# chinhau5/parallel_eda

Hardware: AMD Instinct MI355X
Metric: place+route wall-clock to feasibility (s/flow; bitcoin_miner-scale synthetic on stratixiv-like fabric) (lower is better)
Workload: dtype fp32; 1 GPU; model=bitcoin_miner, arch=bitcoin_stratixiv, grid=280x200, W=300, rr_nodes=15745036, rr_edges=87277236, blocks=37632, nets=35616, conns=110426, global_batch=110426, seq_len=0, final_overused=0, wirelength=4914365

## Files before the change

csrc/hip/place_kernel.hip:

```cpp
#include "pnr_hip.h"

namespace pnrh {

struct PlaceDev {
  const int32_t* net_blk_ptr;
  const int32_t* net_blks;
  const int32_t* blk_net_ptr;
  const int32_t* blk_nets;
  const int8_t* blk_type;
  const int8_t* tile_btype;
  const int32_t* type_cols;
  const int32_t* type_col_ptr;
  const uint8_t* fixed;
  const float* net_q;
  const int32_t* net_sink_ptr;
  const float* conn_crit;
  const float* delay_mat;
  int32_t* bx;
  int32_t* by;
  int32_t* bslot;
  int32_t* grid;
  float* net_cost;
  float* net_tcost;
  int32_t num_blocks, num_nets, gx, gy, cap, nx, ny, io_cap;
// ... 390 lines not shown
  }
}

__launch_bounds__(64 * PROP_WAVES, 2)
__global__ void place_apply_kernel(PlaceDev p, MovesDev m, float timing_tradeoff,
                                   double* cost_acc ) {
  const int lane = threadIdx.x & 63;
  const int i = blockIdx.x * PROP_WAVES + (threadIdx.x >> 6);
  if (i >= m.n_moves || m.mv_flags[i] != 2) return;
  int32_t blk = m.mv_blk[i];
  int32_t other = m.mv_other[i];
  int32_t to = m.mv_to[i];
  if (other <= -2) {
    const int mid = -2 - other;
    const int ddx = (to >> 13) - 4096, ddy = (to & 0x1FFF) - 4096;
    const int32_t mm0 = p.macro_ptr[mid], mm1 = p.macro_ptr[mid + 1];
    for (int32_t j = mm0; j < mm1; ++j) {
      int32_t b = p.macro_blk[j];
      for (int32_t k = p.blk_net_ptr[b] + lane; k < p.blk_net_ptr[b + 1];
           k += 64) {
        int32_t n = p.blk_nets[k];
        p.net_cost[n] = net_bb_cost_macro(p, n, mid, ddx, ddy);
        if (timing_tradeoff > 0.0f)
          p.net_tcost[n] = net_td_cost_macro(p, n, mid, ddx, ddy);
      }
    }
    if (lane == 0) {
      for (int32_t j = mm0; j < mm1; ++j) {
        int32_t b = p.macro_blk[j];
        p.grid[((int64_t)p.bx[b] * p.gy + p.by[b]) * p.cap + p.bslot[b]] = -1;
      }
      for (int32_t j = mm0; j < mm1; ++j) {
        int32_t b = p.macro_blk[j];
        int tx = p.bx[b] + ddx, ty = p.by[b] + ddy;
        p.grid[((int64_t)tx * p.gy + ty) * p.cap] = b;
        p.bx[b] = tx; p.by[b] = ty; p.bslot[b] = 0;
      }
      unsafeAtomicAdd(&cost_acc[0], (double)m.mv_dbb[i]);
      unsafeAtomicAdd(&cost_acc[1], (double)m.mv_dtd[i]);
    }
    return;
  }
  int slot1 = to % p.cap;
  int x1 = to / p.cap / p.gy, y1 = (to / p.cap) % p.gy;
  int x0 = p.bx[blk], y0 = p.by[blk], s0 = p.bslot[blk];
  const int ox = other >= 0 ? x0 : -1000, oy = other >= 0 ? y0 : -1000;
  for (int32_t k = p.blk_net_ptr[blk] + lane; k < p.blk_net_ptr[blk + 1];
       k += 64) {
    int32_t n = p.blk_nets[k];
    p.net_cost[n] = net_bb_cost(p, n, blk, x1, y1, other, ox, oy);
    if (timing_tradeoff > 0.0f)
      p.net_tcost[n] = net_td_cost(p, n, blk, x1, y1, other, ox, oy);
  }
  if (other >= 0)
    for (int32_t k = p.blk_net_ptr[other] + lane;
         k < p.blk_net_ptr[other + 1]; k += 64) {
      int32_t n = p.blk_nets[k];
      p.net_cost[n] = net_bb_cost(p, n, blk, x1, y1, other, ox, oy);
      if (timing_tradeoff > 0.0f)
        p.net_tcost[n] = net_td_cost(p, n, blk, x1, y1, other, ox, oy);
    }
  if (lane == 0) {
    p.grid[((int64_t)x0 * p.gy + y0) * p.cap + s0] = other >= 0 ? other : -1;
    p.grid[((int64_t)x1 * p.gy + y1) * p.cap + slot1] = blk;
    p.bx[blk] = x1; p.by[blk] = y1; p.bslot[blk] = slot1;
    if (other >= 0) { p.bx[other] = x0; p.by[other] = y0; p.bslot[other] = s0; }
    unsafeAtomicAdd(&cost_acc[0], (double)m.mv_dbb[i]);
    unsafeAtomicAdd(&cost_acc[1], (double)m.mv_dtd[i]);
  }
}

__global__ void place_reset_claims_kernel(int32_t* net_claim, int32_t nn,
                                          int32_t* loc_claim, int32_t nl,
                                          int32_t* counters) {
  int i = blockIdx.x * blockDim.x + threadIdx.x;
  int total = max(nn, nl);
  (void)counters;
  for (; i < total; i += gridDim.x * blockDim.x) {
    if (i < nn) net_claim[i] = 0x7FFFFFFF;
    if (i < nl) loc_claim[i] = 0x7FFFFFFF;
  }
}

struct RunDev {
  int32_t* mv_from;
  unsigned long long* net_claim;
  unsigned long long* loc_claim;
  int32_t* ctrl;
};

__device__ __forceinline__ unsigned long long claim_key(uint32_t batch, int i) {
  return ((unsigned long long)batch << 32) | (0xFFFFFFFFu - (uint32_t)i);
}

__launch_bounds__(64 * PROP_WAVES, 2)
__global__ void place_propose_run_kernel(PlaceDev p, MovesDev m, RunDev r,
                                         float T, int rlim,
                                         float timing_tradeoff,
                                         float inv_bb_norm, float inv_td_norm,
                                         uint32_t seed, uint32_t batch) {
  if (r.ctrl[0]) return;
  const int lane = threadIdx.x & 63;
  const int i = blockIdx.x * PROP_WAVES + (threadIdx.x >> 6);
  if (i >= m.n_moves) return;
  const unsigned long long key = claim_key(batch, i);
  int sel = -1, sx1 = -1, sy1 = -1, sslot = 0;
  if (lane == 0) {
    m.mv_flags[i] = 0;
    sel = propose_select_impl(p, rlim, seed, batch, i, sx1, sy1, sslot);
  }
  sel = __shfl(sel, 0);
  if (sel < 0) return;
  const int x1 = __shfl(sx1, 0);
  const int y1 = __shfl(sy1, 0);
  const int slot1 = __shfl(sslot, 0);
  const int32_t blk = sel;
  const int x0 = p.bx[blk], y0 = p.by[blk];
  const int mid = p.macro_of ? p.macro_of[blk] : -1;
  if (mid >= 0) {
    const int ddx = x1 - x0, ddy = y1 - y0;
    const int32_t mm0 = p.macro_ptr[mid], mm1 = p.macro_ptr[mid + 1];
    if (mm1 - mm0 > 16) return;
    int ok = 0;
    if (lane == 0) {
      ok = 1;
      for (int32_t j = mm0; j < mm1 && ok; ++j) {
        int32_t b = p.macro_blk[j];
        int sx = p.bx[b], sy = p.by[b];
        int tx = sx + ddx, ty = sy + ddy;
        if (p.fixed && p.fixed[b]) ok = 0;
        else if (tx < 0 || tx >= p.gx || ty < 0 || ty >= p.gy) ok = 0;
        else if (p.rx0 >= 0 && (tx < p.rx0 || tx > p.rx1 ||
                                sx < p.rx0 || sx > p.rx1)) ok = 0;
        else if (p.tile_btype
                     ? (p.tile_btype[tx * p.gy + ty] != p.blk_type[b])
                     : (is_io_loc(p, tx, ty) != (p.blk_type[b] == 0))) ok = 0;
        else if (cap_at(p, tx, ty) != 1) ok = 0;
        else {
          int32_t occ = p.grid[((int64_t)tx * p.gy + ty) * p.cap];
          if (occ >= 0 && p.macro_of[occ] != mid) ok = 0;
        }
      }
      if (ok) atomicAdd(&m.counters[0], 1);
    }
    ok = __shfl(ok, 0);
    if (!ok) return;
    float dbb = 0.0f, dtd = 0.0f;
    for (int32_t j = mm0; j < mm1; ++j) {
      int32_t b = p.macro_blk[j];
      for (int32_t k = p.blk_net_ptr[b] + lane; k < p.blk_net_ptr[b + 1];
           k += 64) {
        int32_t n = p.blk_nets[k];
        bool dup = false;
        for (int32_t j2 = mm0; j2 < j && !dup; ++j2)
          dup = blk_has_net(p, p.macro_blk[j2], n);
        if (dup) continue;
        dbb += net_bb_cost_macro(p, n, mid, ddx, ddy) - p.net_cost[n];
        if (timing_tradeoff > 0.0f)
          dtd += net_td_cost_macro(p, n, mid, ddx, ddy) - p.net_tcost[n];
      }
    }
    dbb = wave_sum_f32(dbb);
    dtd = wave_sum_f32(dtd);
    float delta = (1.0f - timing_tradeoff) * dbb * inv_bb_norm +
                  timing_tradeoff * dtd * inv_td_norm;
    bool accept;
    if (delta <= 0.0f) accept = true;
    else if (T <= 0.0f) accept = false;
    else {
      float u = (rng_hash(seed, batch, i * 131 + 5) & 0xFFFFFF) *
                (1.0f / 16777216.0f);
      accept = u < __expf(-delta / T);
    }
    if (!accept) return;
    if (lane == 0) {
      atomicAdd(&m.counters[1], 1);
      m.mv_blk[i] = blk;
      m.mv_to[i] = ((ddx + 4096) << 13) | (ddy + 4096);
      m.mv_other[i] = -2 - mid;
      m.mv_dbb[i] = dbb;
      m.mv_dtd[i] = dtd;
      m.mv_flags[i] = 1;
      r.mv_from[i] = x0 * p.gy + y0;
    }
    for (int32_t j = mm0; j < mm1; ++j) {
      int32_t b = p.macro_blk[j];
      for (int32_t k = p.blk_net_ptr[b] + lane; k < p.blk_net_ptr[b + 1];
           k += 64)
        atomicMax(&r.net_claim[p.blk_nets[k]], key);
    }
    for (int32_t j = mm0 + lane; j < mm1; j += 64) {
      int32_t b = p.macro_blk[j];
      atomicMax(&r.loc_claim[p.bx[b] * p.gy + p.by[b]], key);
      atomicMax(&r.loc_claim[(p.bx[b] + ddx) * p.gy + p.by[b] + ddy], key);
    }
    return;
  }
  int32_t other = p.grid[((int64_t)x1 * p.gy + y1) * p.cap + slot1];
  if (other == blk) return;
  if (other >= 0 && p.fixed && p.fixed[other]) return;
  if (other >= 0 && p.macro_of && p.macro_of[other] >= 0)
    return;
  if (lane == 0) atomicAdd(&m.counters[0], 1);
  float dbb = 0.0f, dtd = 0.0f;
  const int ox = other >= 0 ? x0 : -1000, oy = other >= 0 ? y0 : -1000;
  for (int32_t k = p.blk_net_ptr[blk] + lane; k < p.blk_net_ptr[blk + 1];
       k += 64) {
    int32_t n = p.blk_nets[k];
    dbb += net_bb_cost(p, n, blk, x1, y1, other, ox, oy) - p.net_cost[n];
    if (timing_tradeoff > 0.0f)
      dtd += net_td_cost(p, n, blk, x1, y1, other, ox, oy) - p.net_tcost[n];
  }
  if (other >= 0) {
    for (int32_t k = p.blk_net_ptr[other] + lane;
         k < p.blk_net_ptr[other + 1]; k += 64) {
      int32_t n = p.blk_nets[k];
      if (blk_has_net(p, blk, n)) continue;
      dbb += net_bb_cost(p, n, blk, x1, y1, other, ox, oy) - p.net_cost[n];
      if (timing_tradeoff > 0.0f)
        dtd += net_td_cost(p, n, blk, x1, y1, other, ox, oy) - p.net_tcost[n];
    }
  }
  dbb = wave_sum_f32(dbb);
  dtd = wave_sum_f32(dtd);
  float delta = (1.0f - timing_tradeoff) * dbb * inv_bb_norm +
                timing_tradeoff * dtd * inv_td_norm;
  bool accept;
  if (delta <= 0.0f) accept = true;
  else if (T <= 0.0f) accept = false;
  else {
    float u = (rng_hash(seed, batch, i * 131 + 5) & 0xFFFFFF) *
              (1.0f / 16777216.0f);
    accept = u < __expf(-delta / T);
  }
  if (!accept) return;
  if (lane == 0) {
    atomicAdd(&m.counters[1], 1);
    m.mv_blk[i] = blk;
    m.mv_to[i] = ((x1 * p.gy + y1) * p.cap + slot1);
    m.mv_other[i] = other;
    m.mv_dbb[i] = dbb;
    m.mv_dtd[i] = dtd;
    m.mv_flags[i] = 1;
    r.mv_from[i] = x0 * p.gy + y0;
    atomicMax(&r.loc_claim[x0 * p.gy + y0], key);
    atomicMax(&r.loc_claim[x1 * p.gy + y1], key);
  }
  for (int32_t k = p.blk_net_ptr[blk] + lane; k < p.blk_net_ptr[blk + 1];
       k += 64)
    atomicMax(&r.net_claim[p.blk_nets[k]], key);
  if (other >= 0)
    for (int32_t k = p.blk_net_ptr[other] + lane;
         k < p.blk_net_ptr[other + 1]; k += 64)
      atomicMax(&r.net_claim[p.blk_nets[k]], key);
}

__device__ void commit_move(const PlaceDev& p, const MovesDev& m,
                            const RunDev& r, float timing_tradeoff,
                            double* cost_acc, uint32_t batch) {
  const int lane = threadIdx.x & 63;
  const int i = blockIdx.x * PROP_WAVES + (threadIdx.x >> 6);
  if (i >= m.n_moves || m.mv_flags[i] != 1) return;
  const unsigned long long key = claim_key(batch, i);
  int32_t blk = m.mv_blk[i];
  int32_t other = m.mv_other[i];
  int32_t to = m.mv_to[i];
  bool bad = false;
  if (other <= -2) {
    const int mid = -2 - other;
    const int ddx = (to >> 13) - 4096, ddy = (to & 0x1FFF) - 4096;
    const int32_t mm0 = p.macro_ptr[mid], mm1 = p.macro_ptr[mid + 1];
    for (int32_t j = mm0 + lane; j < mm1; j += 64) {
      int32_t b = p.macro_blk[j];
      int sx = p.bx[b], sy = p.by[b];
      int tx = sx + ddx, ty = sy + ddy;
      if (tx < 0 || tx >= p.gx || ty < 0 || ty >= p.gy) bad = true;
      else if (r.loc_claim[sx * p.gy + sy] != key ||
               r.loc_claim[tx * p.gy + ty] != key) bad = true;
    }
    for (int32_t j = mm0; j < mm1; ++j) {
      int32_t b = p.macro_blk[j];
      for (int32_t k = p.blk_net_ptr[b] + lane; k < p.blk_net_ptr[b + 1];
           k += 64)
        if (r.net_claim[p.blk_nets[k]] != key) bad = true;
    }
  } else {
    int x1 = to / p.cap / p.gy, y1 = (to / p.cap) % p.gy;
    if (lane == 0 && (r.loc_claim[r.mv_from[i]] != key ||
                      r.loc_claim[x1 * p.gy + y1] != key)) bad = true;
    for (int32_t k = p.blk_net_ptr[blk] + lane; k < p.blk_net_ptr[blk + 1];
         k += 64)
      if (r.net_claim[p.blk_nets[k]] != key) bad = true;
    if (other >= 0)
      for (int32_t k = p.blk_net_ptr[other] + lane;
           k < p.blk_net_ptr[other + 1]; k += 64)
        if (r.net_claim[p.blk_nets[k]] != key) bad = true;
  }
  const bool win = !__any(bad);
  if (lane == 0) {
    if (!win) { m.mv_flags[i] = 0; atomicAdd(&m.counters[3], 1); }
    else { m.mv_flags[i] = 2; atomicAdd(&m.counters[2], 1); }
  }
  if (!win) return;
  if (other <= -2) {
    const int mid = -2 - other;
    const int ddx = (to >> 13) - 4096, ddy = (to & 0x1FFF) - 4096;
    const int32_t mm0 = p.macro_ptr[mid], mm1 = p.macro_ptr[mid + 1];
    for (int32_t j = mm0; j < mm1; ++j) {
      int32_t b = p.macro_blk[j];
      for (int32_t k = p.blk_net_ptr[b] + lane; k < p.blk_net_ptr[b + 1];
           k += 64) {
        int32_t n = p.blk_nets[k];
        p.net_cost[n] = net_bb_cost_macro(p, n, mid, ddx, ddy);
        if (timing_tradeoff > 0.0f)
          p.net_tcost[n] = net_td_cost_macro(p, n, mid, ddx, ddy);
      }
    }
    if (lane == 0) {
      for (int32_t j = mm0; j < mm1; ++j) {
        int32_t b = p.macro_blk[j];
        p.grid[((int64_t)p.bx[b] * p.gy + p.by[b]) * p.cap + p.bslot[b]] = -1;
      }
      for (int32_t j = mm0; j < mm1; ++j) {
        int32_t b = p.macro_blk[j];
        int tx = p.bx[b] + ddx, ty = p.by[b] + ddy;
        p.grid[((int64_t)tx * p.gy + ty) * p.cap] = b;
        p.bx[b] = tx; p.by[b] = ty; p.bslot[b] = 0;
      }
      unsafeAtomicAdd(&cost_acc[0], (double)m.mv_dbb[i]);
      unsafeAtomicAdd(&cost_acc[1], (double)m.mv_dtd[i]);
    }
    return;
  }
  int slot1 = to % p.cap;
  int x1 = to / p.cap / p.gy, y1 = (to / p.cap) % p.gy;
  int x0 = p.bx[blk], y0 = p.by[blk], s0 = p.bslot[blk];
  const int ox = other >= 0 ? x0 : -1000, oy = other >= 0 ? y0 : -1000;
  for (int32_t k = p.blk_net_ptr[blk] + lane; k < p.blk_net_ptr[blk + 1];
       k += 64) {
    int32_t n = p.blk_nets[k];
    p.net_cost[n] = net_bb_cost(p, n, blk, x1, y1, other, ox, oy);
    if (timing_tradeoff > 0.0f)
      p.net_tcost[n] = net_td_cost(p, n, blk, x1, y1, other, ox, oy);
  }
  if (other >= 0)
    for (int32_t k = p.blk_net_ptr[other] + lane;
         k < p.blk_net_ptr[other + 1]; k += 64) {
      int32_t n = p.blk_nets[k];
      p.net_cost[n] = net_bb_cost(p, n, blk, x1, y1, other, ox, oy);
      if (timing_tradeoff > 0.0f)
        p.net_tcost[n] = net_td_cost(p, n, blk, x1, y1, other, ox, oy);
    }
  if (lane == 0) {
    p.grid[((int64_t)x0 * p.gy + y0) * p.cap + s0] = other >= 0 ? other : -1;
    p.grid[((int64_t)x1 * p.gy + y1) * p.cap + slot1] = blk;
    p.bx[blk] = x1; p.by[blk] = y1; p.bslot[blk] = slot1;
    if (other >= 0) { p.bx[other] = x0; p.by[other] = y0; p.bslot[other] = s0; }
    unsafeAtomicAdd(&cost_acc[0], (double)m.mv_dbb[i]);
    unsafeAtomicAdd(&cost_acc[1], (double)m.mv_dtd[i]);
  }
}

__launch_bounds__(64 * PROP_WAVES, 2)
__global__ void place_commit_kernel(PlaceDev p, MovesDev m, RunDev r,
                                    float timing_tradeoff, double* cost_acc,
                                    uint32_t batch, int check,
                                    int32_t target_moves) {
  if (r.ctrl[0]) return;
  commit_move(p, m, r, timing_tradeoff, cost_acc, batch);
  if (!check) return;
  asm volatile("s_waitcnt vmcnt(0)" ::: "memory");
  __syncthreads();
  if (threadIdx.x != 0) return;
  __threadfence();
  asm volatile("s_waitcnt vmcnt(0)" ::: "memory");
  int ticket = __hip_atomic_fetch_add(&r.ctrl[2], 1, __ATOMIC_RELAXED,
                                      __HIP_MEMORY_SCOPE_AGENT);
  if (ticket != (int)gridDim.x - 1) return;
  __threadfence();
  int att = __hip_atomic_load(&m.counters[0], __ATOMIC_RELAXED,
                              __HIP_MEMORY_SCOPE_AGENT);
  int acc = __hip_atomic_load(&m.counters[1], __ATOMIC_RELAXED,
                              __HIP_MEMORY_SCOPE_AGENT);
  int win = __hip_atomic_load(&m.counters[2], __ATOMIC_RELAXED,
                              __HIP_MEMORY_SCOPE_AGENT);
  r.ctrl[1] += 4;
  if (win + (att - acc) >= target_moves) r.ctrl[0] = 1;
  __hip_atomic_store(&r.ctrl[2], 0, __ATOMIC_RELAXED,
                     __HIP_MEMORY_SCOPE_AGENT);
}

__global__ void place_refresh_costs_kernel(PlaceDev p, float timing_tradeoff,
                                           double* out ) {
  int n = blockIdx.x * blockDim.x + threadIdx.x;
  for (; n < p.num_nets; n += gridDim.x * blockDim.x) {
    float c = net_bb_cost(p, n, -1, 0, 0, -1, 0, 0);
    p.net_cost[n] = c;
    unsafeAtomicAdd(&out[0], (double)c);
    float t = (timing_tradeoff > 0.0f)
                  ? net_td_cost(p, n, -1, 0, 0, -1, 0, 0) : 0.0f;
    p.net_tcost[n] = t;
    unsafeAtomicAdd(&out[1], (double)t);
  }
}

}

using namespace pnrh;

extern "C" {

struct PlaceLaunchArgs {
  const int32_t* net_blk_ptr; const int32_t* net_blks;
  const int32_t* blk_net_ptr; const int32_t* blk_nets;
  const int8_t* blk_type; const int8_t* tile_btype;
  const int32_t* type_cols; const int32_t* type_col_ptr;
  const uint8_t* fixed;
  const float* net_q;
  const int32_t* net_sink_ptr; const float* conn_crit; const float* delay_mat;
  int32_t* bx; int32_t* by; int32_t* bslot; int32_t* grid;
  float* net_cost; float* net_tcost;
  int32_t num_blocks, num_nets, gx, gy, cap, nx, ny, io_cap;
  int32_t rx0, rx1;
  const int32_t* macro_of; const int32_t* macro_ptr;
  const int32_t* macro_blk;
  int32_t* mv_blk; int32_t* mv_to; int32_t* mv_other;
  float* mv_dbb; float* mv_dtd; uint8_t* mv_flags;
  int32_t* net_claim; int32_t* loc_claim; int32_t* counters;
  int32_t n_moves;
  float T; int32_t rlim; float timing_tradeoff;
  float inv_bb_norm, inv_td_norm;
  uint32_t seed, batch;
  double* cost_acc;
  int32_t* mv_from;
  unsigned long long* net_claim64; unsigned long long* loc_claim64;
  int32_t* run_ctrl;
};

static void unpack(const PlaceLaunchArgs* a, PlaceDev& p, MovesDev& m) {
  p.net_blk_ptr = a->net_blk_ptr; p.net_blks = a->net_blks;
  p.blk_net_ptr = a->blk_net_ptr; p.blk_nets = a->blk_nets;
  p.blk_type = a->blk_type; p.tile_btype = a->tile_btype;
  p.type_cols = a->type_cols; p.type_col_ptr = a->type_col_ptr;
  p.fixed = a->fixed;
  p.net_q = a->net_q;
  p.net_sink_ptr = a->net_sink_ptr; p.conn_crit = a->conn_crit;
  p.delay_mat = a->delay_mat;
  p.bx = a->bx; p.by = a->by; p.bslot = a->bslot; p.grid = a->grid;
  p.net_cost = a->net_cost; p.net_tcost = a->net_tcost;
  p.num_blocks = a->num_blocks; p.num_nets = a->num_nets;
  p.gx = a->gx; p.gy = a->gy; p.cap = a->cap;
  p.nx = a->nx; p.ny = a->ny; p.io_cap = a->io_cap;
  p.rx0 = a->rx0; p.rx1 = a->rx1;
  p.macro_of = a->macro_of; p.macro_ptr = a->macro_ptr;
  p.macro_blk = a->macro_blk;
  m.mv_blk = a->mv_blk; m.mv_to = a->mv_to; m.mv_other = a->mv_other;
  m.mv_dbb = a->mv_dbb; m.mv_dtd = a->mv_dtd; m.mv_flags = a->mv_flags;
  m.net_claim = a->net_claim; m.loc_claim = a->loc_claim;
  m.counters = a->counters; m.n_moves = a->n_moves;
}

int pnr_place_batch(const PlaceLaunchArgs* a, void* stream) {
  PlaceDev p; MovesDev m;
  unpack(a, p, m);
  hipStream_t s = (hipStream_t)stream;
  int rg = (max(max(a->num_nets, a->gx * a->gy), a->n_moves) + 255) / 256;
  rg = rg < 2048 ? rg : 2048;
  hipLaunchKernelGGL(place_reset_claims_kernel, dim3(rg), dim3(256), 0, s,
                     m.net_claim, p.num_nets, m.loc_claim, p.gx * p.gy,
                     m.counters);
  int mg = (m.n_moves + PROP_WAVES - 1) / PROP_WAVES;
  hipLaunchKernelGGL(place_propose_kernel, dim3(mg), dim3(64 * PROP_WAVES),
                     0, s, p, m, a->T, a->rlim, a->timing_tradeoff,
                     a->inv_bb_norm, a->inv_td_norm, a->seed, a->batch);
  hipLaunchKernelGGL(place_resolve_kernel, dim3(mg), dim3(64 * PROP_WAVES),
                     0, s, p, m);
  hipLaunchKernelGGL(place_apply_kernel, dim3(mg), dim3(64 * PROP_WAVES),
                     0, s, p, m, a->timing_tradeoff, a->cost_acc);
  return (int)hipGetLastError();
}

int pnr_place_run(const PlaceLaunchArgs* a, uint32_t first_batch,
                  int32_t target_moves, int32_t n_batches, void* stream) {
  if (n_batches < 0 || (n_batches & 3) || first_batch == 0 ||
      !a->mv_from || !a->net_claim64 || !a->loc_claim64 || !a->run_ctrl)
    return (int)hipErrorInvalidValue;
  PlaceDev p; MovesDev m;
  unpack(a, p, m);
  RunDev r;
  r.mv_from = a->mv_from;
  r.net_claim = a->net_claim64; r.loc_claim = a->loc_claim64;
  r.ctrl = a->run_ctrl;
  hipStream_t s = (hipStream_t)stream;
  int mg = (m.n_moves + PROP_WAVES - 1) / PROP_WAVES;
  for (int32_t k = 0; k < n_batches; ++k) {
    const uint32_t batch = first_batch + (uint32_t)k;
    hipLaunchKernelGGL(place_propose_run_kernel, dim3(mg),
                       dim3(64 * PROP_WAVES), 0, s, p, m, r, a->T, a->rlim,
                       a->timing_tradeoff, a->inv_bb_norm, a->inv_td_norm,
                       a->seed, batch);
    hipLaunchKernelGGL(place_commit_kernel, dim3(mg), dim3(64 * PROP_WAVES),
                       0, s, p, m, r, a->timing_tradeoff, a->cost_acc, batch,
                       (int)(((k + 1) & 3) == 0), target_moves);
  }
  return (int)hipGetLastError();
}

int pnr_place_refresh(const PlaceLaunchArgs* a, void* stream) {
  PlaceDev p; MovesDev m;
  unpack(a, p, m);
  hipStream_t s = (hipStream_t)stream;
  hipLaunchKernelGGL(place_refresh_costs_kernel, dim3(1024), dim3(256), 0, s,
                     p, a->timing_tradeoff, a->cost_acc);
  return (int)hipGetLastError();
}

int64_t pnr_place_args_sizeof() { return (int64_t)sizeof(PlaceLaunchArgs); }

}
```

parallel_eda_amd/place/gpu_placer.py:

```python
import ctypes as ct
import math

import numpy as np

from ..arch.archdef import ArchDef
from ..ops import hip_api
from .placer import Placement, analytic_delay_matrix


class PlaceLaunchArgs(ct.Structure):
    _fields_ = [
        ("net_blk_ptr", ct.c_void_p), ("net_blks", ct.c_void_p),
        ("blk_net_ptr", ct.c_void_p), ("blk_nets", ct.c_void_p),
        ("blk_type", ct.c_void_p), ("tile_btype", ct.c_void_p),
        ("type_cols", ct.c_void_p), ("type_col_ptr", ct.c_void_p),
        ("fixed", ct.c_void_p),
        ("net_q", ct.c_void_p),
        ("net_sink_ptr", ct.c_void_p), ("conn_crit", ct.c_void_p),
        ("delay_mat", ct.c_void_p),
        ("bx", ct.c_void_p), ("by", ct.c_void_p), ("bslot", ct.c_void_p),
        ("grid", ct.c_void_p),
        ("net_cost", ct.c_void_p), ("net_tcost", ct.c_void_p),
        ("num_blocks", ct.c_int32), ("num_nets", ct.c_int32),
        ("gx", ct.c_int32), ("gy", ct.c_int32), ("cap", ct.c_int32),
        ("nx", ct.c_int32), ("ny", ct.c_int32), ("io_cap", ct.c_int32),
        ("rx0", ct.c_int32), ("rx1", ct.c_int32),
        ("macro_of", ct.c_void_p), ("macro_ptr", ct.c_void_p),
        ("macro_blk", ct.c_void_p),
        ("mv_blk", ct.c_void_p), ("mv_to", ct.c_void_p), ("mv_other", ct.c_void_p),
        ("mv_dbb", ct.c_void_p), ("mv_dtd", ct.c_void_p), ("mv_flags", ct.c_void_p),
        ("net_claim", ct.c_void_p), ("loc_claim", ct.c_void_p),
        ("counters", ct.c_void_p), ("n_moves", ct.c_int32),
        ("T", ct.c_float), ("rlim", ct.c_int32), ("timing_tradeoff", ct.c_float),
        ("inv_bb_norm", ct.c_float), ("inv_td_norm", ct.c_float),
        ("seed", ct.c_uint32), ("batch", ct.c_uint32),
        ("cost_acc", ct.c_void_p),
        ("mv_from", ct.c_void_p),
        ("net_claim64", ct.c_void_p), ("loc_claim64", ct.c_void_p),
        ("run_ctrl", ct.c_void_p),
    ]


RUN_CHUNK_BATCHES = 32


def _lib():
    lib = hip_api.lib()
    if not hasattr(lib, "_place_ready"):
        lib.pnr_place_batch.restype = ct.c_int
        lib.pnr_place_batch.argtypes = [ct.POINTER(PlaceLaunchArgs), ct.c_void_p]
        lib.pnr_place_run.restype = ct.c_int
        lib.pnr_place_run.argtypes = [ct.POINTER(PlaceLaunchArgs), ct.c_uint32,
                                      ct.c_int32, ct.c_int32, ct.c_void_p]
        lib.pnr_place_refresh.restype = ct.c_int
        lib.pnr_place_refresh.argtypes = [ct.POINTER(PlaceLaunchArgs), ct.c_void_p]
        lib.pnr_place_args_sizeof.restype = ct.c_int64
        if lib.pnr_place_args_sizeof() != ct.sizeof(PlaceLaunchArgs):
            raise RuntimeError("PlaceLaunchArgs ABI mismatch")
        lib._place_ready = True
    return lib


def ptr(t):
    return ct.c_void_p(t.data_ptr())


class GpuPlacer:
    def __init__(self, netlist, arch: ArchDef, seed=7, timing=False,
                 device="cuda:0", n_moves=None, fixed=None,
                 delay_matrix="analytic", macros=None, legacy_batches=False):
        import torch
        self.torch = torch
        self.legacy_batches = legacy_batches
        self.device = device
        self.arch = arch
        self.nl = netlist
        self.seed = seed
        self.timing = timing
        nb = netlist.num_blocks
        nn = netlist.num_nets
        gx, gy = arch.nx + 2, arch.ny + 2
        self.gx, self.gy = gx, gy
        self.cap = max(1, arch.io_cap)
        self.batch_counter = 0

        counts = 1 + np.diff(netlist.net_sink_ptr)
        net_blk_ptr = np.r_[0, np.cumsum(counts)].astype(np.int32)
        net_blks = np.empty(net_blk_ptr[-1], dtype=np.int32)
        net_blks[net_blk_ptr[:-1]] = netlist.net_driver
        is_sink = np.ones(len(net_blks), dtype=bool)
        is_sink[net_blk_ptr[:-1]] = False
        net_blks[is_sink] = netlist.net_sinks
        net_of_member = np.repeat(np.arange(nn, dtype=np.int64),
                                  np.diff(net_blk_ptr))
        key = net_blks.astype(np.int64) * nn + net_of_member
        key = np.unique(key)
        mb = (key // nn).astype(np.int32)
        blk_nets = (key % nn).astype(np.int32)
        blk_net_ptr = np.zeros(nb + 1, dtype=np.int32)
        np.add.at(blk_net_ptr, mb + 1, 1)
        blk_net_ptr = np.cumsum(blk_net_ptr, dtype=np.int64).astype(np.int32)
        q = _cross_count_vec(counts).astype(np.float32)

        def up(a, dtype=None):
            t = torch.from_numpy(np.ascontiguousarray(a))
            return t.to(device)

        self.t_net_blk_ptr = up(net_blk_ptr)
        self.t_net_blks = up(net_blks)
        self.t_blk_net_ptr = up(blk_net_ptr)
        self.t_blk_nets = up(blk_nets)
        self.t_blk_type = up(netlist.block_type)
        self.t_tile_btype = (up(arch.tile_btype_grid())
                             if arch.is_heterogeneous() else None)
        self.t_type_cols = self.t_type_col_ptr = None
        if arch.is_heterogeneous():
            ram_cols = [x for x in range(1, arch.nx + 1)
                        if arch.col_block_type(x) == 2]
            dsp_cols = [x for x in range(1, arch.nx + 1)
                        if arch.col_block_type(x) == 3]
            self.t_type_cols = up(np.asarray(ram_cols + dsp_cols,
                                             dtype=np.int32))
            self.t_type_col_ptr = up(np.asarray(
                [0, len(ram_cols), len(ram_cols) + len(dsp_cols)],
                dtype=np.int32))
        self.t_net_q = up(q)
        self._fixed = fixed
        self.t_fixed = None
        if fixed is not None:
            mask = np.zeros(nb, dtype=np.uint8)
            mask[np.asarray(fixed[0], dtype=np.int64)] = 1
            self.t_fixed = up(mask)
        self.t_net_sink_ptr = up(netlist.net_sink_ptr.astype(np.int32))
        self.t_conn_crit = torch.zeros(netlist.num_conns, dtype=torch.float32,
                                       device=device)
        if timing:
            if delay_matrix == "routed":
                from .delay_matrix import routed_delay_matrix
                dm = routed_delay_matrix(arch)
            else:
                dm = analytic_delay_matrix(arch)
            self._dm = dm
            self.t_delay_mat = up(dm.ravel())
        else:
            self._dm = None
            self.t_delay_mat = None

        bx, by, bslot, grid = self._initial_placement(seed)
        self.t_macro_of = self.t_macro_ptr = self.t_macro_blk = None
        self.macros = macros or []
        if self.macros:
            bx, by, bslot, grid = self._legalize_macros(
                bx, by, bslot, grid, self.macros)
            macro_of = np.full(nb, -1, dtype=np.int32)
            mptr = [0]
            mblk = []
            for mi, grp in enumerate(self.macros):
                for (b, dx, dy) in grp:
                    macro_of[b] = mi
                    mblk.append(b)
                mptr.append(len(mblk))
            self.t_macro_of = up(macro_of)
            self.t_macro_ptr = up(np.asarray(mptr, dtype=np.int32))
            self.t_macro_blk = up(np.asarray(mblk, dtype=np.int32))
        self.t_bx = up(bx); self.t_by = up(by); self.t_bslot = up(bslot)
        self.t_grid = up(grid)
        self.t_net_cost = torch.zeros(nn, dtype=torch.float32, device=device)
        self.t_net_tcost = torch.zeros(nn, dtype=torch.float32, device=device)

        self.n_moves = n_moves or int(np.clip(nb // 16, 64, 1 << 16))
        nm = self.n_moves
        self.t_mv_blk = torch.zeros(nm, dtype=torch.int32, device=device)
        self.t_mv_to = torch.zeros(nm, dtype=torch.int32, device=device)
        self.t_mv_other = torch.zeros(nm, dtype=torch.int32, device=device)
        self.t_mv_dbb = torch.zeros(nm, dtype=torch.float32, device=device)
        self.t_mv_dtd = torch.zeros(nm, dtype=torch.float32, device=device)
        self.t_mv_flags = torch.zeros(nm, dtype=torch.uint8, device=device)
        self.t_net_claim = self.t_loc_claim = None
        self.t_net_claim64 = self.t_loc_claim64 = None
        if legacy_batches:
            self.t_net_claim = torch.zeros(nn, dtype=torch.int32, device=device)
            self.t_loc_claim = torch.zeros(gx * gy, dtype=torch.int32,
                                           device=device)
        else:
            self.t_net_claim64 = torch.zeros(nn, dtype=torch.int64,
                                             device=device)
            self.t_loc_claim64 = torch.zeros(gx * gy, dtype=torch.int64,
                                             device=device)
        self.t_mv_from = torch.zeros(nm, dtype=torch.int32, device=device)
        self.t_run_state = torch.zeros(8, dtype=torch.int32, device=device)
        self.t_counters = self.t_run_state[:4]
        self.t_run_ctrl = self.t_run_state[4:]
        self.t_cost_acc = torch.zeros(2, dtype=torch.float64, device=device)

        self.lib = _lib()
        self.bb_cost, self.td_cost = self.refresh_costs()

    def _initial_placement(self, seed):
        arch = self.arch
        nl = self.nl
        rng = np.random.default_rng(seed)
        nb = nl.num_blocks
        bx = np.zeros(nb, dtype=np.int32)
        by = np.zeros(nb, dtype=np.int32)
        bslot = np.zeros(nb, dtype=np.int32)
        if self._fixed is not None:
            bx2, by2, bs2, grid = self._initial_placement_free(rng)
            ids, fx, fy, fs = [np.asarray(a) for a in self._fixed]
            for b, x, y, sl in zip(ids, fx, fy, fs):
                occ = grid[x, y, sl]
                if occ == b:
                    continue
                grid[bx2[b], by2[b], bs2[b]] = occ
                if occ >= 0:
                    bx2[occ], by2[occ], bs2[occ] = bx2[b], by2[b], bs2[b]
                bx2[b], by2[b], bs2[b] = x, y, sl
                grid[x, y, sl] = b
            return bx2, by2, bs2, grid.reshape(-1)
        return self._initial_placement_free(rng, flat=True)

    def _legalize_macros(self, bx, by, bslot, grid, macros):
        arch = self.arch
        g = grid.reshape(self.gx, self.gy, self.cap)
        members = [b for grp in macros for (b, _, _) in grp]
        for b in members:
            g[bx[b], by[b], bslot[b]] = -1
        tb = (arch.tile_btype_grid().reshape(self.gx, self.gy)
              if arch.is_heterogeneous() else None)

        def tile_ok(b, x, y):
            if not (0 <= x < self.gx and 0 <= y < self.gy):
                return False
            bt = int(self.nl.block_type[b])
            if tb is not None:
                if tb[x, y] != bt:
                    return False
            else:
                io = (x == 0 or x == self.gx - 1 or
                      y == 0 or y == self.gy - 1)
                inner = 1 <= x <= arch.nx and 1 <= y <= arch.ny
                if bt == 0 or io or not inner:
                    return False
            return g[x, y, 0] < 0

        for grp in macros:
            placed = False
            for ax in range(1, arch.nx + 1):
                for ay in range(1, arch.ny + 1):
                    if all(tile_ok(b, ax + dx, ay + dy)
                           for (b, dx, dy) in grp):
                        for (b, dx, dy) in grp:
                            bx[b], by[b], bslot[b] = ax + dx, ay + dy, 0
                            g[ax + dx, ay + dy, 0] = b
                        placed = True
                        break
                if placed:
                    break
            if not placed:
                raise ValueError("cannot legalize macro (grid too full)")
        return bx, by, bslot, g.reshape(-1)

    def _initial_placement_free(self, rng, flat=False):
        arch = self.arch
        nl = self.nl
        nb = nl.num_blocks
        bx = np.zeros(nb, dtype=np.int32)
        by = np.zeros(nb, dtype=np.int32)
        bslot = np.zeros(nb, dtype=np.int32)
        grid = np.full((self.gx, self.gy, self.cap), -1, dtype=np.int32)
        ios = np.nonzero(nl.block_type == 0)[0]
        if not arch.is_heterogeneous():
            clbs = np.nonzero(nl.block_type == 1)[0]
            tiles = rng.permutation(arch.nx * arch.ny)[:len(clbs)]
            if len(tiles) < len(clbs):
                raise ValueError("too many CLBs for grid")
            bx[clbs] = tiles // arch.ny + 1
            by[clbs] = tiles % arch.ny + 1
            grid[bx[clbs], by[clbs], 0] = clbs
        else:
            col_t = np.asarray([arch.col_block_type(x)
                                for x in range(1, arch.nx + 1)])
            for t in (1, 2, 3):
                blks = np.nonzero(nl.block_type == t)[0]
                if not len(blks):
                    continue
                cols = np.nonzero(col_t == t)[0]
                cand = (cols[:, None] * arch.ny +
                        np.arange(arch.ny)[None, :]).ravel()
                if len(blks) > len(cand):
                    raise ValueError(f"too many type-{t} blocks for grid")
                tiles = cand[rng.permutation(len(cand))[:len(blks)]]
                bx[blks] = tiles // arch.ny + 1
                by[blks] = tiles % arch.ny + 1
                grid[bx[blks], by[blks], 0] = blks
        io_locs = ([(0, y) for y in range(1, arch.ny + 1)] +
                   [(self.gx - 1, y) for y in range(1, arch.ny + 1)] +
                   [(x, 0) for x in range(1, arch.nx + 1)] +
                   [(x, self.gy - 1) for x in range(1, arch.nx + 1)])
        slots = [(x, y, s) for (x, y) in io_locs for s in range(arch.io_cap)]
        sel = rng.permutation(len(slots))[:len(ios)]
        for b, k in zip(ios, sel):
            x, y, s = slots[k]
            bx[b], by[b], bslot[b] = x, y, s
            grid[x, y, s] = b
        return (bx, by, bslot, grid.reshape(-1)) if flat \
            else (bx, by, bslot, grid)

    def _args(self, T=0.0, rlim=1, tt=0.0, inv_bb=1.0, inv_td=1.0):
        a = PlaceLaunchArgs()
        a.net_blk_ptr = ptr(self.t_net_blk_ptr); a.net_blks = ptr(self.t_net_blks)
        a.blk_net_ptr = ptr(self.t_blk_net_ptr); a.blk_nets = ptr(self.t_blk_nets)
        a.blk_type = ptr(self.t_blk_type)
        a.tile_btype = (ptr(self.t_tile_btype)
                        if self.t_tile_btype is not None else None)
        a.type_cols = (ptr(self.t_type_cols)
                       if self.t_type_cols is not None else None)
        a.type_col_ptr = (ptr(self.t_type_col_ptr)
                          if self.t_type_col_ptr is not None else None)
        a.fixed = ptr(self.t_fixed) if self.t_fixed is not None else None
        a.net_q = ptr(self.t_net_q)
        a.net_sink_ptr = ptr(self.t_net_sink_ptr)
        a.conn_crit = ptr(self.t_conn_crit)
        a.delay_mat = ptr(self.t_delay_mat) if self.t_delay_mat is not None else None
        a.bx = ptr(self.t_bx); a.by = ptr(self.t_by); a.bslot = ptr(self.t_bslot)
        a.grid = ptr(self.t_grid)
        a.net_cost = ptr(self.t_net_cost); a.net_tcost = ptr(self.t_net_tcost)
        a.num_blocks = self.nl.num_blocks; a.num_nets = self.nl.num_nets
        a.gx = self.gx; a.gy = self.gy; a.cap = self.cap
        a.nx = self.arch.nx; a.ny = self.arch.ny; a.io_cap = self.arch.io_cap
        a.rx0, a.rx1 = getattr(self, "move_region", (-1, -1))
        if getattr(self, "t_macro_of", None) is not None:
            a.macro_of = ptr(self.t_macro_of)
            a.macro_ptr = ptr(self.t_macro_ptr)
            a.macro_blk = ptr(self.t_macro_blk)
        else:
            a.macro_of = a.macro_ptr = a.macro_blk = None
        a.mv_blk = ptr(self.t_mv_blk); a.mv_to = ptr(self.t_mv_to)
        a.mv_other = ptr(self.t_mv_other); a.mv_dbb = ptr(self.t_mv_dbb)
        a.mv_dtd = ptr(self.t_mv_dtd); a.mv_flags = ptr(self.t_mv_flags)
        if self.legacy_batches:
            a.net_claim = ptr(self.t_net_claim)
            a.loc_claim = ptr(self.t_loc_claim)
            a.net_claim64 = a.loc_claim64 = None
        else:
            a.net_claim = a.loc_claim = None
            a.net_claim64 = ptr(self.t_net_claim64)
            a.loc_claim64 = ptr(self.t_loc_claim64)
        a.mv_from = ptr(self.t_mv_from)
        a.run_ctrl = ptr(self.t_run_ctrl)
        a.counters = ptr(self.t_counters); a.n_moves = self.n_moves
        a.T = T; a.rlim = max(1, int(rlim)); a.timing_tradeoff = tt
        a.inv_bb_norm = inv_bb; a.inv_td_norm = inv_td
        a.seed = self.seed & 0xFFFFFFFF; a.batch = self.batch_counter
        a.cost_acc = ptr(self.t_cost_acc)
        return a

    def _stream(self):
        return self.torch.cuda.current_stream().cuda_stream

    def refresh_costs(self):
        self.t_cost_acc.zero_()
        a = self._args(tt=1.0 if self.timing else 0.0)
        rc = self.lib.pnr_place_refresh(ct.byref(a), self._stream())
        hip_api.check(rc, "place_refresh")
        self.torch.cuda.synchronize(self.device)
        bb, td = self.t_cost_acc.cpu().numpy()
        self.bb_cost, self.td_cost = float(bb), float(td)
        return self.bb_cost, self.td_cost

    def run_batches(self, T, rlim, target_moves, tt, bb_norm, td_norm,
                    max_batches=256):
        if self.legacy_batches:
            return self._run_batches_legacy(T, rlim, target_moves, tt,
                                            bb_norm, td_norm, max_batches)
        self.t_run_state.zero_()
        a = self._args(T=T, rlim=rlim, tt=tt,
                       inv_bb=1.0 / bb_norm, inv_td=1.0 / td_norm)
        target = int(min(max(math.ceil(target_moves), -0x7FFFFFFF),
                         0x7FFFFFFF))
        cap = 4 * ((max_batches + 3) // 4)
        first = self.batch_counter + 1
        enq = 0
        att = acc = executed = 0
        while enq < cap:
            n = min(RUN_CHUNK_BATCHES, cap - enq)
            rc = self.lib.pnr_place_run(ct.byref(a), first + enq, target, n,
                                        self._stream())
            hip_api.check(rc, "place_run")
            enq += n
            st = self.t_run_state.cpu().numpy()
            att, acc = int(st[0]), int(st[1])
            done, executed = int(st[4]), int(st[5])
            if done:
                break
        self.batch_counter += executed
        srate = acc / max(1, att)
        return srate, att

    def _run_batches_legacy(self, T, rlim, target_moves, tt, bb_norm, td_norm,
                            max_batches=256):
        self.t_counters.zero_()
        batches = 0
        win = att = acc = 0
        while batches < max_batches:
            for _ in range(4):
                self.batch_counter += 1
                a = self._args(T=T, rlim=rlim, tt=tt,
                               inv_bb=1.0 / bb_norm, inv_td=1.0 / td_norm)
                rc = self.lib.pnr_place_batch(ct.byref(a), self._stream())
                hip_api.check(rc, "place_batch")
                batches += 1
            self.torch.cuda.synchronize(self.device)
            c = self.t_counters.cpu().numpy()
            att, acc, win = int(c[0]), int(c[1]), int(c[2])
            if win + (att - acc) >= target_moves:
                break
        else:
            self.torch.cuda.synchronize(self.device)
        srate = acc / max(1, att)
        return srate, att

    def set_move_region(self, x0, x1):
        self.move_region = (x0, x1)

    def set_crit(self, conn_crit):
        t = self.torch.from_numpy(np.ascontiguousarray(conn_crit,
                                                       dtype=np.float32))
        self.t_conn_crit.copy_(t.to(self.device))

    def placement(self):
# ... 144 lines not shown
```

Baseline: 7.774 s.

## Flatten move evaluation into per-pin LDS work and cache new net costs for commit

For swap moves whose blocks have at most 64 nets and 256 total pins, the propose kernel now assigns one net per lane and spreads all pins of the affected nets across the wave. It builds bounding boxes with LDS atomics and collects criticality/delay pairs in LDS, replacing a serial per-net walk in each lane. The recomputed net costs are stored in per-move row buffers so commit copies them instead of re-running net_bb_cost/net_td_cost. This adds per-move global buffers and an LDS footprint that may reduce occupancy, and keeps the old path as a fallback for large moves.

```diff
diff --git a/csrc/hip/place_kernel.hip b/csrc/hip/place_kernel.hip
--- a/csrc/hip/place_kernel.hip
+++ b/csrc/hip/place_kernel.hip
@@ -496,15 +496,75 @@
   }
 }
 
+#define EVAL_MAX_NETS 64
+#define EVAL_MAX_PAIRS 256
+#define EVAL_SLOTS (2 * EVAL_MAX_NETS)
+
 struct RunDev {
   int32_t* mv_from;
   unsigned long long* net_claim;
   unsigned long long* loc_claim;
   int32_t* ctrl;
+  int32_t* mv_walk;
+  float* row_cost;
+  float* row_tcost;
+  unsigned long long* row_mask;
+};
+
+struct EvalLds {
+  int32_t e0[EVAL_SLOTS];
+  int32_t c0[EVAL_SLOTS];
+  int32_t start[EVAL_SLOTS];
+  int32_t xmin[EVAL_SLOTS], xmax[EVAL_SLOTS];
+  int32_t ymin[EVAL_SLOTS], ymax[EVAL_SLOTS];
+  float2 cd[EVAL_MAX_PAIRS];
+  uint8_t slot[EVAL_MAX_PAIRS];
 };
 
 __device__ __forceinline__ unsigned long long claim_key(uint32_t batch, int i) {
   return ((unsigned long long)batch << 32) | (0xFFFFFFFFu - (uint32_t)i);
+}
+
+__device__ __forceinline__ void wave_lds_sync() {
+  __builtin_amdgcn_fence(__ATOMIC_RELEASE, "wavefront");
+  __builtin_amdgcn_wave_barrier();
+  __builtin_amdgcn_fence(__ATOMIC_ACQUIRE, "wavefront");
+}
+
+__device__ __forceinline__ int wave_incl_scan_i32(int v, int lane) {
+  for (int off = 1; off < 64; off <<= 1) {
+    int t = __shfl_up(v, off);
+    if (lane >= off) v += t;
+  }
+  return v;
+}
+
+__device__ __forceinline__ void eval_open_slot(EvalLds& L, int s, int32_t e0,
+                                               int32_t c0, int start, int len) {
+  L.e0[s] = e0; L.c0[s] = c0; L.start[s] = start;
+  L.xmin[s] = 1 << 28; L.xmax[s] = -1;
+  L.ymin[s] = 1 << 28; L.ymax[s] = -1;
+  for (int j = 0; j < len; ++j) L.slot[start + j] = (uint8_t)s;
+}
+
+__device__ __forceinline__ void eval_close_slot(
+    const EvalLds& L, int s, int start, int len, float q, float old_cost,
+    float old_tcost, bool tt_on, bool have_dm, float& dbb, float& dtd,
+    float& new_cost, float& new_tcost) {
+  const int span = (L.xmax[s] - L.xmin[s] + 1) + (L.ymax[s] - L.ymin[s] + 1);
+  const float fs = (float)span;
+  new_cost = __fmul_rn(q, fs);
+  dbb += fmaf(q, fs, -old_cost);
+  if (tt_on) {
+    float t = 0.0f;
+    if (have_dm)
+      for (int j = 1; j < len; ++j) {
+        const float2 cd = L.cd[start + j];
+        t = fmaf(cd.x, cd.y, t);
+      }
+    new_tcost = t;
+    dtd += t - old_tcost;
+  }
 }
 
 __launch_bounds__(64 * PROP_WAVES, 2)
@@ -523,11 +583,11 @@
     m.mv_flags[i] = 0;
     sel = propose_select_impl(p, rlim, seed, batch, i, sx1, sy1, sslot);
   }
-  sel = __shfl(sel, 0);
+  sel = __builtin_amdgcn_readfirstlane(sel);
   if (sel < 0) return;
-  const int x1 = __shfl(sx1, 0);
-  const int y1 = __shfl(sy1, 0);
-  const int slot1 = __shfl(sslot, 0);
+  const int x1 = __builtin_amdgcn_readfirstlane(sx1);
+  const int y1 = __builtin_amdgcn_readfirstlane(sy1);
+  const int slot1 = __builtin_amdgcn_readfirstlane(sslot);
   const int32_t blk = sel;
   const int x0 = p.bx[blk], y0 = p.by[blk];
   const int mid = p.macro_of ? p.macro_of[blk] : -1;
@@ -596,6 +656,7 @@
       m.mv_dtd[i] = dtd;
       m.mv_flags[i] = 1;
       r.mv_from[i] = x0 * p.gy + y0;
+      r.mv_walk[i] = 1;
     }
     for (int32_t j = mm0; j < mm1; ++j) {
       int32_t b = p.macro_blk[j];
@@ -618,16 +679,92 @@
   if (lane == 0) atomicAdd(&m.counters[0], 1);
   float dbb = 0.0f, dtd = 0.0f;
   const int ox = other >= 0 ? x0 : -1000, oy = other >= 0 ? y0 : -1000;
-  for (int32_t k = p.blk_net_ptr[blk] + lane; k < p.blk_net_ptr[blk + 1];
-       k += 64) {
-    int32_t n = p.blk_nets[k];
-    dbb += net_bb_cost(p, n, blk, x1, y1, other, ox, oy) - p.net_cost[n];
-    if (timing_tradeoff > 0.0f)
-      dtd += net_td_cost(p, n, blk, x1, y1, other, ox, oy) - p.net_tcost[n];
-  }
-  if (other >= 0) {
-    for (int32_t k = p.blk_net_ptr[other] + lane;
-         k < p.blk_net_ptr[other + 1]; k += 64) {
+  const bool tt_on = timing_tradeoff > 0.0f;
+  const int32_t pb = p.blk_net_ptr[blk];
+  const int nb = p.blk_net_ptr[blk + 1] - pb;
+  const int32_t po = other >= 0 ? p.blk_net_ptr[other] : 0;
+  const int no = other >= 0 ? p.blk_net_ptr[other + 1] - po : 0;
+  int32_t nA = -1, nO = -1, e0A = 0, e0O = 0, c0A = 0, c0O = 0;
+  int lenA = 0, lenO = 0, startA = 0, startO = 0, total = 0;
+  float qA = 0.0f, qO = 0.0f, oldA = 0.0f, oldO = 0.0f;
+  float oldtA = 0.0f, oldtO = 0.0f;
+  float newA = 0.0f, newO = 0.0f, newtA = 0.0f, newtO = 0.0f;
+  bool evalO = false;
+  bool fast = nb <= EVAL_MAX_NETS && no <= EVAL_MAX_NETS;
+  if (fast) {
+    if (lane < nb) nA = p.blk_nets[pb + lane];
+    if (lane < no) nO = p.blk_nets[po + lane];
+    bool shared = false;
+    for (int j = 0; j < nb; ++j)
+      shared |= nO == __builtin_amdgcn_readlane(nA, j);
+    evalO = nO >= 0 && !shared;
+    if (nA >= 0) {
+      e0A = p.net_blk_ptr[nA]; lenA = p.net_blk_ptr[nA + 1] - e0A;
+      c0A = p.net_sink_ptr[nA];
+      qA = p.net_q[nA]; oldA = p.net_cost[nA];
+      if (tt_on) oldtA = p.net_tcost[nA];
+    }
+    if (evalO) {
+      e0O = p.net_blk_ptr[nO]; lenO = p.net_blk_ptr[nO + 1] - e0O;
+      c0O = p.net_sink_ptr[nO];
+      qO = p.net_q[nO]; oldO = p.net_cost[nO];
+      if (tt_on) oldtO = p.net_tcost[nO];
+    }
+    const int cA = min(lenA, EVAL_MAX_PAIRS + 1);
+    const int cO = min(lenO, EVAL_MAX_PAIRS + 1);
+    const int inc = wave_incl_scan_i32(cA | (cO << 16), lane);
+    const int tot = __shfl(inc, 63);
+    const int totA = tot & 0xFFFF;
+    total = totA + (tot >> 16);
+    startA = (inc & 0xFFFF) - cA;
+    startO = totA + (inc >> 16) - cO;
+    fast = total <= EVAL_MAX_PAIRS;
+  }
+  if (fast) {
+    __shared__ EvalLds lds[PROP_WAVES];
+    EvalLds& L = lds[threadIdx.x >> 6];
+    const bool have_dm = p.delay_mat != nullptr;
+    if (nA >= 0) eval_open_slot(L, lane, e0A, c0A, startA, lenA);
+    if (evalO)
+      eval_open_slot(L, EVAL_MAX_NETS + lane, e0O, c0O, startO, lenO);
+    wave_lds_sync();
+    for (int base = 0; base < total; base += 64) {
+      const int f = base + lane;
+      if (f >= total) continue;
+      const int s = L.slot[f];
+      const int32_t e0 = L.e0[s];
+      const int j = f - L.start[s];
+      const int32_t b = p.net_blks[e0 + j];
+      int x = p.bx[b], y = p.by[b];
+      if (b == blk) { x = x1; y = y1; }
+      else if (b == other) { x = ox; y = oy; }
+      atomicMin(&L.xmin[s], x); atomicMax(&L.xmax[s], x);
+      atomicMin(&L.ymin[s], y); atomicMax(&L.ymax[s], y);
+      if (tt_on && have_dm && j > 0) {
+        const int32_t drv = p.net_blks[e0];
+        int dx0 = p.bx[drv], dy0 = p.by[drv];
+        if (drv == blk) { dx0 = x1; dy0 = y1; }
+        else if (drv == other) { dx0 = ox; dy0 = oy; }
+        const int dx = abs(x - dx0), dy = abs(y - dy0);
+        L.cd[f] = make_float2(p.conn_crit[L.c0[s] + (j - 1)],
+                              p.delay_mat[dx * p.gy + dy]);
+      }
+    }
+    wave_lds_sync();
+    if (nA >= 0)
+      eval_close_slot(L, lane, startA, lenA, qA, oldA, oldtA, tt_on, have_dm,
+                      dbb, dtd, newA, newtA);
+    if (evalO)
+      eval_close_slot(L, EVAL_MAX_NETS + lane, startO, lenO, qO, oldO, oldtO,
+                      tt_on, have_dm, dbb, dtd, newO, newtO);
+  } else {
+    for (int32_t k = pb + lane; k < pb + nb; k += 64) {
+      int32_t n = p.blk_nets[k];
+      dbb += net_bb_cost(p, n, blk, x1, y1, other, ox, oy) - p.net_cost[n];
+      if (timing_tradeoff > 0.0f)
+        dtd += net_td_cost(p, n, blk, x1, y1, other, ox, oy) - p.net_tcost[n];
+    }
+    for (int32_t k = po + lane; k < po + no; k += 64) {
       int32_t n = p.blk_nets[k];
       if (blk_has_net(p, blk, n)) continue;
       dbb += net_bb_cost(p, n, blk, x1, y1, other, ox, oy) - p.net_cost[n];
@@ -657,16 +794,31 @@
     m.mv_dtd[i] = dtd;
     m.mv_flags[i] = 1;
     r.mv_from[i] = x0 * p.gy + y0;
+    r.mv_walk[i] = fast ? 0 : 1;
     atomicMax(&r.loc_claim[x0 * p.gy + y0], key);
     atomicMax(&r.loc_claim[x1 * p.gy + y1], key);
   }
-  for (int32_t k = p.blk_net_ptr[blk] + lane; k < p.blk_net_ptr[blk + 1];
-       k += 64)
+  if (fast) {
+    const unsigned long long mask = __ballot(evalO);
+    float* rc = r.row_cost + (size_t)i * EVAL_SLOTS;
+    float* rt = r.row_tcost + (size_t)i * EVAL_SLOTS;
+    if (lane == 0) r.row_mask[i] = mask;
+    if (nA >= 0) {
+      rc[lane] = newA;
+      if (tt_on) rt[lane] = newtA;
+      atomicMax(&r.net_claim[nA], key);
+    }
+    if (evalO) {
+      rc[EVAL_MAX_NETS + lane] = newO;
+      if (tt_on) rt[EVAL_MAX_NETS + lane] = newtO;
+    }
+    if (nO >= 0) atomicMax(&r.net_claim[nO], key);
+    return;
+  }
+  for (int32_t k = pb + lane; k < pb + nb; k += 64)
     atomicMax(&r.net_claim[p.blk_nets[k]], key);
-  if (other >= 0)
-    for (int32_t k = p.blk_net_ptr[other] + lane;
-         k < p.blk_net_ptr[other + 1]; k += 64)
-      atomicMax(&r.net_claim[p.blk_nets[k]], key);
+  for (int32_t k = po + lane; k < po + no; k += 64)
+    atomicMax(&r.net_claim[p.blk_nets[k]], key);
 }
 
 __device__ void commit_move(const PlaceDev& p, const MovesDev& m,
@@ -680,6 +832,10 @@
   int32_t other = m.mv_other[i];
   int32_t to = m.mv_to[i];
   bool bad = false;
+  bool rows = false;
+  int32_t nA = -1, nO = -1;
+  int32_t pb = 0, po = 0;
+  int nb = 0, no = 0;
   if (other <= -2) {
     const int mid = -2 - other;
     const int ddx = (to >> 13) - 4096, ddy = (to & 0x1FFF) - 4096;
@@ -702,13 +858,22 @@
     int x1 = to / p.cap / p.gy, y1 = (to / p.cap) % p.gy;
     if (lane == 0 && (r.loc_claim[r.mv_from[i]] != key ||
                       r.loc_claim[x1 * p.gy + y1] != key)) bad = true;
-    for (int32_t k = p.blk_net_ptr[blk] + lane; k < p.blk_net_ptr[blk + 1];
-         k += 64)
-      if (r.net_claim[p.blk_nets[k]] != key) bad = true;
-    if (other >= 0)
-      for (int32_t k = p.blk_net_ptr[other] + lane;
-           k < p.blk_net_ptr[other + 1]; k += 64)
+    rows = r.mv_walk[i] == 0;
+    pb = p.blk_net_ptr[blk]; nb = p.blk_net_ptr[blk + 1] - pb;
+    if (other >= 0) {
+      po = p.blk_net_ptr[other]; no = p.blk_net_ptr[other + 1] - po;
+    }
+    if (rows) {
+      if (lane < nb) nA = p.blk_nets[pb + lane];
+      if (lane < no) nO = p.blk_nets[po + lane];
+      if (nA >= 0 && r.net_claim[nA] != key) bad = true;
+      if (nO >= 0 && r.net_claim[nO] != key) bad = true;
+    } else {
+      for (int32_t k = pb + lane; k < pb + nb; k += 64)
         if (r.net_claim[p.blk_nets[k]] != key) bad = true;
+      for (int32_t k = po + lane; k < po + no; k += 64)
+        if (r.net_claim[p.blk_nets[k]] != key) bad = true;
+    }
   }
   const bool win = !__any(bad);
   if (lane == 0) {
@@ -750,21 +915,32 @@
   int x1 = to / p.cap / p.gy, y1 = (to / p.cap) % p.gy;
   int x0 = p.bx[blk], y0 = p.by[blk], s0 = p.bslot[blk];
   const int ox = other >= 0 ? x0 : -1000, oy = other >= 0 ? y0 : -1000;
-  for (int32_t k = p.blk_net_ptr[blk] + lane; k < p.blk_net_ptr[blk + 1];
-       k += 64) {
-    int32_t n = p.blk_nets[k];
-    p.net_cost[n] = net_bb_cost(p, n, blk, x1, y1, other, ox, oy);
-    if (timing_tradeoff > 0.0f)
-      p.net_tcost[n] = net_td_cost(p, n, blk, x1, y1, other, ox, oy);
-  }
-  if (other >= 0)
-    for (int32_t k = p.blk_net_ptr[other] + lane;
-         k < p.blk_net_ptr[other + 1]; k += 64) {
+  if (rows) {
+    const float* rc = r.row_cost + (size_t)i * EVAL_SLOTS;
+    const float* rt = r.row_tcost + (size_t)i * EVAL_SLOTS;
+    const bool evalO = nO >= 0 && ((r.row_mask[i] >> lane) & 1ull);
+    if (nA >= 0) {
+      p.net_cost[nA] = rc[lane];
+      if (timing_tradeoff > 0.0f) p.net_tcost[nA] = rt[lane];
+    }
+    if (evalO) {
+      p.net_cost[nO] = rc[EVAL_MAX_NETS + lane];
+      if (timing_tradeoff > 0.0f) p.net_tcost[nO] = rt[EVAL_MAX_NETS + lane];
+    }
+  } else {
+    for (int32_t k = pb + lane; k < pb + nb; k += 64) {
       int32_t n = p.blk_nets[k];
       p.net_cost[n] = net_bb_cost(p, n, blk, x1, y1, other, ox, oy);
       if (timing_tradeoff > 0.0f)
         p.net_tcost[n] = net_td_cost(p, n, blk, x1, y1, other, ox, oy);
     }
+    for (int32_t k = po + lane; k < po + no; k += 64) {
+      int32_t n = p.blk_nets[k];
+      p.net_cost[n] = net_bb_cost(p, n, blk, x1, y1, other, ox, oy);
+      if (timing_tradeoff > 0.0f)
+        p.net_tcost[n] = net_td_cost(p, n, blk, x1, y1, other, ox, oy);
+    }
+  }
   if (lane == 0) {
     p.grid[((int64_t)x0 * p.gy + y0) * p.cap + s0] = other >= 0 ? other : -1;
     p.grid[((int64_t)x1 * p.gy + y1) * p.cap + slot1] = blk;
@@ -849,6 +1025,9 @@
   int32_t* mv_from;
   unsigned long long* net_claim64; unsigned long long* loc_claim64;
   int32_t* run_ctrl;
+  int32_t* mv_walk;
+  float* row_cost; float* row_tcost;
+  unsigned long long* row_mask;
 };
 
 static void unpack(const PlaceLaunchArgs* a, PlaceDev& p, MovesDev& m) {
@@ -897,7 +1076,8 @@
 int pnr_place_run(const PlaceLaunchArgs* a, uint32_t first_batch,
                   int32_t target_moves, int32_t n_batches, void* stream) {
   if (n_batches < 0 || (n_batches & 3) || first_batch == 0 ||
-      !a->mv_from || !a->net_claim64 || !a->loc_claim64 || !a->run_ctrl)
+      !a->mv_from || !a->net_claim64 || !a->loc_claim64 || !a->run_ctrl ||
+      !a->mv_walk || !a->row_cost || !a->row_tcost || !a->row_mask)
     return (int)hipErrorInvalidValue;
   PlaceDev p; MovesDev m;
   unpack(a, p, m);
@@ -905,6 +1085,9 @@
   r.mv_from = a->mv_from;
   r.net_claim = a->net_claim64; r.loc_claim = a->loc_claim64;
   r.ctrl = a->run_ctrl;
+  r.mv_walk = a->mv_walk;
+  r.row_cost = a->row_cost; r.row_tcost = a->row_tcost;
+  r.row_mask = a->row_mask;
   hipStream_t s = (hipStream_t)stream;
   int mg = (m.n_moves + PROP_WAVES - 1) / PROP_WAVES;
   for (int32_t k = 0; k < n_batches; ++k) {
@@ -931,4 +1114,8 @@
 
 int64_t pnr_place_args_sizeof() { return (int64_t)sizeof(PlaceLaunchArgs); }
 
-}
+int32_t pnr_place_eval_max_nets() { return EVAL_MAX_NETS; }
+int32_t pnr_place_eval_max_pairs() { return EVAL_MAX_PAIRS; }
+int32_t pnr_place_eval_row_slots() { return EVAL_SLOTS; }
+
+}
diff --git a/parallel_eda_amd/place/gpu_placer.py b/parallel_eda_amd/place/gpu_placer.py
--- a/parallel_eda_amd/place/gpu_placer.py
+++ b/parallel_eda_amd/place/gpu_placer.py
@@ -38,6 +38,9 @@
         ("mv_from", ct.c_void_p),
         ("net_claim64", ct.c_void_p), ("loc_claim64", ct.c_void_p),
         ("run_ctrl", ct.c_void_p),
+        ("mv_walk", ct.c_void_p),
+        ("row_cost", ct.c_void_p), ("row_tcost", ct.c_void_p),
+        ("row_mask", ct.c_void_p),
     ]
 
 
@@ -55,10 +58,20 @@
         lib.pnr_place_refresh.restype = ct.c_int
         lib.pnr_place_refresh.argtypes = [ct.POINTER(PlaceLaunchArgs), ct.c_void_p]
         lib.pnr_place_args_sizeof.restype = ct.c_int64
+        for f in ("pnr_place_eval_max_nets", "pnr_place_eval_max_pairs",
+                  "pnr_place_eval_row_slots"):
+            getattr(lib, f).restype = ct.c_int32
+            getattr(lib, f).argtypes = []
         if lib.pnr_place_args_sizeof() != ct.sizeof(PlaceLaunchArgs):
             raise RuntimeError("PlaceLaunchArgs ABI mismatch")
         lib._place_ready = True
     return lib
+
+
+def eval_caps():
+    lib = _lib()
+    return (int(lib.pnr_place_eval_max_nets()),
+            int(lib.pnr_place_eval_max_pairs()))
 
 
 def ptr(t):
@@ -188,6 +201,17 @@
             self.t_loc_claim64 = torch.zeros(gx * gy, dtype=torch.int64,
                                              device=device)
         self.t_mv_from = torch.zeros(nm, dtype=torch.int32, device=device)
+        self.t_mv_walk = self.t_row_cost = self.t_row_tcost = None
+        self.t_row_mask = None
+        if not legacy_batches:
+            slots = int(_lib().pnr_place_eval_row_slots())
+            self.t_mv_walk = torch.zeros(nm, dtype=torch.int32, device=device)
+            self.t_row_cost = torch.zeros(nm * slots, dtype=torch.float32,
+                                          device=device)
+            self.t_row_tcost = torch.zeros(nm * slots, dtype=torch.float32,
+                                           device=device)
+            self.t_row_mask = torch.zeros(nm, dtype=torch.int64,
+                                          device=device)
         self.t_run_state = torch.zeros(8, dtype=torch.int32, device=device)
         self.t_counters = self.t_run_state[:4]
         self.t_run_ctrl = self.t_run_state[4:]
@@ -342,10 +366,15 @@
             a.net_claim = ptr(self.t_net_claim)
             a.loc_claim = ptr(self.t_loc_claim)
             a.net_claim64 = a.loc_claim64 = None
+            a.mv_walk = a.row_cost = a.row_tcost = a.row_mask = None
         else:
             a.net_claim = a.loc_claim = None
             a.net_claim64 = ptr(self.t_net_claim64)
             a.loc_claim64 = ptr(self.t_loc_claim64)
+            a.mv_walk = ptr(self.t_mv_walk)
+            a.row_cost = ptr(self.t_row_cost)
+            a.row_tcost = ptr(self.t_row_tcost)
+            a.row_mask = ptr(self.t_row_mask)
         a.mv_from = ptr(self.t_mv_from)
         a.run_ctrl = ptr(self.t_run_ctrl)
         a.counters = ptr(self.t_counters); a.n_moves = self.n_moves
```

After: 8.003 s. +2.9%, slower.
